# AbbVie-ComputationalGenomics/SAIGEgds

Measured on AMD Instinct MI355X. Metric: variants/sec seqAssocGLMM_SPA at N=430K; achieved HBM GB/s vs roofline, higher is better.
Workload: dtype f64

## Files before the change

### saigegds_amd/csrc/host_lanes.h

```cpp
extern "C" int sgx_set_option(sgx_handle *h, const char *name, long long value)
{
	if (!h || !name) return fail(SGX_EINVAL, "sgx_set_option: NULL argument");
	const std::string n(name);
	if (n == "score_v1") h->force_v1 = value != 0;
	else if (n == "force_dense") h->force_dense = value != 0;
	else if (n == "spa_exact") h->force_exact = value != 0;
	else if (n == "pipe_mb") { if (value < 0 || value > 65536) return fail(SGX_EINVAL, "pipe_mb out of range"); h->pipe_bytes = (size_t)value << 20; return SGX_OK; }
	else if (n == "spa_abl") h->spa_abl = (int)value;
	else if (n == "guard_exp") { if (value < 0 || value > 300) return fail(SGX_EINVAL, "guard_exp must be 0..300"); h->guard_tol = std::pow(10.0, -(double)value); }
	else if (n == "three_plane") { if (value < -1 || value > 1) return fail(SGX_EINVAL, "three_plane must be -1 (automatic), 0 or 1"); h->dense_opt = (int)value; return SGX_OK; }
	else if (n == "lanes") {
		if (value < 1 || value > 4) return fail(SGX_EINVAL, "lanes must be 1..4");
		if (h->owner) return fail(SGX_EINVAL, "lanes: not on a twin");
		int rc = sgx_sync(h);
		if (rc) return rc;
		for (int i = (int)value - 1; i < 3; i++) if (h->twins[i]) { sgx_free(h->twins[i]); h->twins[i] = nullptr; }
		for (int i = 0; i < (int)value - 1; i++) {
			if (h->twins[i]) continue;
			sgx_handle *t = new sgx_handle();
			t->device = h->device; t->md = h->md; t->mf_ok = h->mf_ok; t->mfe = h->mfe;
			for (int g = 0; g < MF_MAXG; g++) { t->mf[g] = h->mf[g]; t->mf_nbfv[g] = h->mf_nbfv[g]; }
			t->dF = h->dF; t->dX = h->dX; t->dy = h->dy; t->dmu = h->dmu; t->dmu2 = h->dmu2; t->dXM = h->dXM; t->dFl = h->dFl; t->dQ = h->dQ;
			t->shares_model = true; t->owner = h;
			t->force_dense = h->force_dense; t->force_v1 = h->force_v1; t->force_exact = h->force_exact;
			t->spa_abl = h->spa_abl; t->guard_tol = h->guard_tol;
			rc = set_dev(t);
			if (!rc) rc = alloc_workspace(t);
			if (rc) { sgx_free(t); return rc; }
			h->twins[i] = t;
		}
		h->n_lanes = (int)value; h->next_lane = 0; h->last_issued = nullptr;
		return SGX_OK;
	}
	else return fail(SGX_EINVAL, "sgx_set_option: unknown option '%s'", name);
	for (sgx_handle *t : h->twins) if (t) { int rc = sgx_set_option(t, name, value); if (rc) return rc; }
	return SGX_OK;
}

static void stats_add(sgx_stats &into, const sgx_stats &x)
{
	into.n_variants += x.n_variants; into.n_valid += x.n_valid; into.n_spa += x.n_spa;
	into.n_spa_dense += x.n_spa_dense; into.n_spa_slow += x.n_spa_slow;
	into.ms_score += x.ms_score; into.ms_spa += x.ms_spa; into.ms_total += x.ms_total;
	into.ms_kernel += x.ms_kernel; into.ms_lists += x.ms_lists;
	into.score_launches += x.score_launches; into.spa_launches += x.spa_launches;
	into.three_plane += x.three_plane; into.n_unlisted += x.n_unlisted; into.n_guarded += x.n_guarded;
}

static int sync_lane(sgx_handle *h)
{
	int rc = set_dev(h);
	if (rc) return rc;
	HIPCHK(hipStreamSynchronize(h->stream));
	if (h->pend_dense.active) {
		h->pend_dense.active = false;
		if (h->stats_pending && h->h_counters[2] > 0) {
			rc = launch_pending_dense(h);
			if (rc) return rc;
			HIPCHK(hipStreamSynchronize(h->stream));
		}
	}
	if (h->stats_pending) {
		h->stats.n_spa = (uint64_t)(h->h_counters[0] + h->h_counters[7] - h->h_counters[6] + h->h_counters[5]);
		h->stats.n_valid = (uint64_t)h->h_counters[1];
		h->stats.n_spa_dense = (uint64_t)h->h_counters[2];
		h->stats.n_spa_slow = (uint64_t)h->h_counters[4];
		h->stats.three_plane = h->form == FORM_THREE ? 1u : 0u;
		h->stats.n_guarded = (uint32_t)h->h_counters[21];
		h->stats.n_unlisted = (uint32_t)h->h_counters[23] - h->stats.n_guarded;
		if (h->form != FORM_FP64) {
			sgx_handle *p = h->owner ? h->owner : h;
			const double frac = 64.0 * (double)h->h_counters[22] / ((double)std::max<uint64_t>(1, h->stats.n_variants) * (double)h->md.N);
			const bool over = (uint64_t)h->stats.n_unlisted * 32 > h->stats.n_variants;
			if (h->form != FORM_THREE && (frac > SGX_DENSE_ON || over)) p->dense_mode = true;
			else if (h->form == FORM_THREE && frac < SGX_DENSE_OFF) p->dense_mode = false;
		}
#ifdef SPA5_PROF
		fprintf(stderr, "routing: tier A %d, tier B %d (of them handed on by A: %d), per-variant kernels %d (series list %d, exact list %d), dense %d\n",
			h->h_counters[0], h->h_counters[7], h->h_counters[6], h->h_counters[5], h->h_counters[3], h->h_counters[4], h->h_counters[2]);
		fprintf(stderr, "spa5 phases (10 ns ticks summed over variants): series kernel %d variants: stage %d count %d index %d gather %d series %d (sweep %d sum %d solve %d) | exact kernel %d variants: stage %d count %d index %d gather %d - sweeps %d\n",
			h->h_counters[3], h->h_counters[8], h->h_counters[9], h->h_counters[10], h->h_counters[11], h->h_counters[12], h->h_counters[13], h->h_counters[14], h->h_counters[15],
			h->h_counters[4], h->h_counters[16], h->h_counters[17], h->h_counters[18], h->h_counters[19], h->h_counters[21]);
#endif
		float a = 0, b = 0, c = 0;
		(void)hipEventElapsedTime(&a, h->ev[0], h->ev[1]);
		(void)hipEventElapsedTime(&b, h->ev[1], h->ev[2]);
		(void)hipEventElapsedTime(&c, h->ev[0], h->ev[2]);
		h->stats.ms_score = a; h->stats.ms_spa = b; h->stats.ms_total = c;
		float k = 0;
		if (h->evk_set) (void)hipEventElapsedTime(&k, h->evk[0], h->evk[1]);
		h->stats.ms_kernel = k; h->evk_set = false;
		float l = 0;
		if (h->lists_timed) { (void)hipEventElapsedTime(&l, h->ev_lists, h->ev[0]); h->stats.ms_total += l; }
		h->stats.ms_lists = l; h->lists_timed = false;
		h->stats_pending = false;
		sgx_handle *p = h->owner ? h->owner : h;
		stats_add(p->total, h->stats);
		p->total_calls++;
	}
	return SGX_OK;
}

extern "C" int sgx_sync(sgx_handle *h)
{
	if (!h) return fail(SGX_EINVAL, "sgx_sync: NULL handle");
	int rc = sync_lane(h);
	for (sgx_handle *t : h->twins) if (!rc && t) rc = sync_lane(t);
	return rc;
}

extern "C" int sgx_get_stats(sgx_handle *h, sgx_stats *st)
{
	if (!h || !st) return fail(SGX_EINVAL, "sgx_get_stats: NULL argument");
	int rc = sgx_sync(h);
	if (rc) return rc;
	*st = (h->last_issued && h->last_issued != h) ? h->last_issued->stats : h->stats;
	return SGX_OK;
}

extern "C" int sgx_get_stats_total(sgx_handle *h, sgx_stats *st, uint64_t *n_calls, int reset)
{
	if (!h || !st) return fail(SGX_EINVAL, "sgx_get_stats_total: NULL argument");
	int rc = sgx_sync(h);
	if (rc) return rc;
	*st = h->total;
	if (n_calls) *n_calls = h->total_calls;
	if (reset) { h->total = sgx_stats{}; h->total_calls = 0; }
	return SGX_OK;
}
```

### saigegds_amd/csrc/host_spa.h

```cpp


template <int LO, typename F, int... I>
static bool with_int(int v, F &&f, std::integer_sequence<int, I...>)
{
	return ((v == LO + I && (f(std::integral_constant<int, LO + I>()), true)) || ...);
}
template <typename F>
static bool with_k(int K, F &&f) { return with_int<1>(K, f, std::make_integer_sequence<int, KMAX>()); }
template <typename F>
static void with_pp(int P, F &&f)
{
	if (P <= 8) f(std::integral_constant<int, 8>());
	else if (P <= 16) f(std::integral_constant<int, 16>());
	else if (P <= 32) f(std::integral_constant<int, 32>());
	else f(std::integral_constant<int, 64>());
}

static dim3 mf_grid(int n_cu, size_t rows, int ntile, int *tps, int vpb = MF_VPB, int wg_per_cu = 2)
{
	const int vt = (int)((rows + vpb - 1) / vpb);
	int sk = std::max(1, (n_cu * wg_per_cu * 4 + vt / 2) / vt);
	sk = std::min(sk, std::max(1, ntile / 24));
	if (sk >= 6) sk = (sk + 7) & ~7;
	sk = std::min(sk, std::max(1, ntile / 2));
	*tps = (ntile + sk - 1) / sk;
	*tps += *tps & 1;
	sk = (ntile + *tps - 1) / *tps;
	return dim3((unsigned)vt, (unsigned)sk);
}

template <int KK, int NCX, int INPUT>
static const void *spa4_moments_fn()
{
	if constexpr (INPUT == IN_2BIT) return (const void *)spa4_moments<KK, NCX>;
	else return (const void *)spa4_moments_ds<KK, NCX, INPUT>;
}

template <int KK, int INPUT>
static int launch_spa_k(sgx_handle *h, RowsRef rr, size_t M, double *out8, bool lazy_dense)
{
	const DevModel &md = h->md;
	constexpr int PB = 512;
	hipStream_t st = h->stream;
	const dim3 sgrid((unsigned)std::min<size_t>(M, (size_t)h->spa_grid));
	if (h->force_v1 && INPUT != IN_2BIT) {
		hipLaunchKernelGGL((spa_kernel<KK, PB, INPUT>), sgrid, dim3(PB), 0, st, rr,
			md, h->recs, h->counters, 0, (const int *)nullptr, h->scratch, h->scratch_stride, out8);
		return SGX_OK;
	}
	const size_t fl = spa4_lds_bytes(KK);
	if (!h->mom_attr_set[INPUT]) {
		HIPCHK(hipFuncSetAttribute(spa4_moments_fn<KK, SPA4_NCA, INPUT>(), hipFuncAttributeMaxDynamicSharedMemorySize, (int)fl));
		HIPCHK(hipFuncSetAttribute(spa4_moments_fn<KK, SPA4_NCB, INPUT>(), hipFuncAttributeMaxDynamicSharedMemorySize, (int)fl));
		h->mom_attr_set[INPUT] = true;
	}
	const int nround = (int)((M + h->vcap4 - 1) / h->vcap4);
	const int btop = (int)(2 * M);
	const dim3 gsolve((unsigned)std::min((h->vcap4 + 3) / 4, 4 * h->n_cu));
	const size_t rowb5 = (size_t)((md.N + 63) / 64) * 16;
	const size_t l5 = (INPUT == IN_2BIT && rowb5 <= 120 * 1024) ? rowb5 : 0;
	const bool small5 = INPUT == IN_2BIT && rowb5 <= 32 * 1024;
	if (l5 > 48 * 1024 && !h->spa5_attr_set[INPUT]) {
		HIPCHK(hipFuncSetAttribute((const void *)spa5_kernel<KK, INPUT, 0, 512>, hipFuncAttributeMaxDynamicSharedMemorySize, (int)l5));
		HIPCHK(hipFuncSetAttribute((const void *)spa5_kernel<KK, INPUT, 1, 512>, hipFuncAttributeMaxDynamicSharedMemorySize, (int)l5));
		h->spa5_attr_set[INPUT] = true;
	}
	const int fx5 = (h->force_exact ? 1 : 0) | (h->spa_abl & ~1);
	auto moments = [&](auto ncx, int tier, int rd) {
		constexpr int NCX = decltype(ncx)::value;
		if constexpr (INPUT == IN_2BIT)
			hipLaunchKernelGGL((spa4_moments<KK, NCX>), dim3((unsigned)h->n_cu), dim3(WAVE * spa4_waves(KK)), fl, st, rr, md, h->nseg,
				tier, btop, rd * h->vcap4, h->vcap4, h->recs, h->counters, h->seg4, h->spa_abl, h->cur5 + 2);
		else
			hipLaunchKernelGGL((spa4_moments_ds<KK, NCX, INPUT>), dim3((unsigned)h->n_cu), dim3(WAVE * spa4_waves(KK)), fl, st,
				(const void *)rr.base, rr.bpv, md, h->nseg, tier, btop, rd * h->vcap4, h->vcap4, h->recs, h->counters, h->seg4, h->cur5 + 2);
		hipLaunchKernelGGL((spa4_solve<KK, NCX>), gsolve, dim3(256), 0, st, md, h->nseg, tier, btop, rd * h->vcap4, h->vcap4,
			h->recs, h->counters, h->seg4, h->fallback, h->fb_x2, out8, h->force_dense ? 1 : 0, h->force_exact ? 1 : 0);
	};
	for (int rd = 0; rd < nround; rd++) moments(std::integral_constant<int, SPA4_NCA>(), 0, rd);
	for (int rd = 0; rd < nround; rd++) moments(std::integral_constant<int, SPA4_NCB>(), 1, rd);
	const int only5 = (INPUT == IN_2BIT && rr.cptr != nullptr && (h->spa_abl & 512)) ? 2 : 0;
	const size_t ws5 = spa5_wg_bytes(md.N);
	auto spa5 = [&](auto threads, int nwg) {
		constexpr int T5 = decltype(threads)::value;
		if constexpr (T5 == 512 || INPUT == IN_2BIT) {
			hipLaunchKernelGGL((spa5_kernel<KK, INPUT, 0, T5>), dim3((unsigned)nwg), dim3(T5), l5, st, rr, md, h->recs, h->counters,
				h->fb_spa2, h->fb_x2, h->cur5, h->fallback, h->scr5, out8, h->force_dense ? 1 : 0, fx5, l5, only5, ws5, 3);
			hipLaunchKernelGGL((spa5_kernel<KK, INPUT, 1, T5>), dim3((unsigned)nwg), dim3(T5), l5, st, rr, md, h->recs, h->counters,
				h->fb_x2, h->fb_x2, h->cur5 + 1, h->fallback, h->scr5, out8, h->force_dense ? 1 : 0, fx5, l5, only5, ws5, 4);
		}
	};
	if (small5) spa5(std::integral_constant<int, 128>(), h->nwg5);
	else spa5(std::integral_constant<int, 512>(), h->n_cu);
	if (!lazy_dense)
		hipLaunchKernelGGL((spa_kernel<KK, PB, INPUT>), sgrid, dim3(PB), 0, st, rr,
			md, h->recs, h->counters, 2, h->fallback, h->scratch, h->scratch_stride, out8);
	return SGX_OK;
}

template <int INPUT>
static int launch_spa(sgx_handle *h, RowsRef rr, size_t M, double *out8, bool lazy_dense = false)
{
	h->stats.spa_launches = 0;
	if (h->md.quant) return SGX_OK;
	int rc = SGX_OK;
	with_k(h->md.K, [&](auto kk) { rc = launch_spa_k<decltype(kk)::value, INPUT>(h, rr, M, out8, lazy_dense); });
	if (rc) return rc;
	HIPCHK(hipGetLastError());
	const bool v1 = h->force_v1 && INPUT != IN_2BIT;
	h->stats.spa_launches = v1 ? 1u : (uint32_t)(4 * ((M + h->vcap4 - 1) / h->vcap4) + 3);
	if (lazy_dense && !v1) { h->pend_dense.active = true; h->pend_dense.rr = rr; h->pend_dense.M = M; h->pend_dense.out8 = out8; }
	return SGX_OK;
}

static int launch_pending_dense(sgx_handle *h)
{
	const dim3 sgrid((unsigned)std::min<size_t>(h->pend_dense.M, (size_t)h->spa_grid));
	with_k(h->md.K, [&](auto kk) {
		hipLaunchKernelGGL((spa_kernel<decltype(kk)::value, 512, IN_2BIT>), sgrid, dim3(512), 0, h->stream, h->pend_dense.rr, h->md,
			h->recs, h->counters, 2, h->fallback, h->scratch, h->scratch_stride, h->pend_dense.out8);
	});
	HIPCHK(hipGetLastError());
	return SGX_OK;
}

static int scan_begin(sgx_handle *h, hipStream_t sst, ScanForm form, const sgx_block *b)
{
	h->form = form;
	if (b) HIPCHK(hipStreamWaitEvent(sst, b->ready, 0));
	if (form == FORM_FP64) {
		HIPCHK(hipMemsetAsync(h->counters, 0, 24 * sizeof(int), sst));
		if (h->cur5) HIPCHK(hipMemsetAsync(h->cur5, 0, 8 * sizeof(int), sst));
	}
	HIPCHK(hipEventRecord(h->ev[0], sst));
	return SGX_OK;
}

template <int INPUT>
static int scan_end(sgx_handle *h, hipStream_t sst, const sgx_block *b, RowsRef rr, size_t M, double *out8, bool lazy_dense)
{
	HIPCHK(hipEventRecord(h->ev[1], sst));
	h->stats.score_launches = h->form == FORM_FP64 ? 1 : 5;
	if (sst != h->stream) HIPCHK(hipStreamWaitEvent(h->stream, h->ev[1], 0));
	int rc = launch_spa<INPUT>(h, rr, M, out8, lazy_dense);
	if (rc) return rc;
	if (lazy_dense) h->pend_dense.blk = b;
	HIPCHK(hipEventRecord(h->ev[2], h->stream));
	if (b) {
		HIPCHK(hipEventRecord(b->last_read, h->stream));
		const_cast<sgx_block *>(b)->was_read = true;
	}
	HIPCHK(hipMemcpyAsync(h->h_counters, h->counters, 24 * sizeof(int), hipMemcpyDeviceToHost, h->stream));
	h->stats.n_variants = M;
	h->stats_pending = true;
	return SGX_OK;
}

template <int KK, int INPUT>
static int launch_score_fp64(sgx_handle *h, RowsRef rr, size_t M, double *out8, uint8_t *valid)
{
	const DevModel &md = h->md;
	constexpr int SB = 256, P = 2 * KK + 2;
	hipStream_t st = h->stream;
	const dim3 grid((unsigned)M);
	if constexpr (INPUT == IN_2BIT) {
		hipLaunchKernelGGL((score2b_kernel<P, SB>), grid, dim3(SB), 0, st,
			rr, (int)M, md, h->recs, h->counters, out8, valid, (const int *)nullptr, 0, 0, (int *)nullptr, (int *)nullptr);
	} else {
		using T = std::conditional_t<INPUT == IN_U8, uint8_t, double>;
		const T *rows = reinterpret_cast<const T *>(rr.base);
		if constexpr (KK <= 8) {
			if (!h->force_v1) {
				const int vb = (int)((M + DS_TILE_VB - 1) / DS_TILE_VB);
				int ns = std::max(1, std::min((4 * h->n_cu + vb - 1) / vb, (md.N + 4095) / 4096));
				int per = (((md.N + ns - 1) / ns) + 63) & ~63;
				ns = (md.N + per - 1) / per;
				const size_t need = (size_t)ns * M * (3 * P + 2) * sizeof(double);
				if (need > h->ds_part_cap) {
					HIPCHK(hipStreamSynchronize(st));
					if (h->ds_part) HIPCHK(hipFree(h->ds_part));
					h->ds_part = nullptr; h->ds_part_cap = 0;
					HIPCHK(hipMalloc((void **)&h->ds_part, need));
					h->ds_part_cap = need;
				}
				hipLaunchKernelGGL((score_ds_tile_kernel<P, T>), dim3((unsigned)vb, (unsigned)ns), dim3(256), 0, st,
					rows, (int)M, md, per, h->ds_part);
				hipLaunchKernelGGL((score_ds_tile_epilogue<P>), dim3((unsigned)((M + 255) / 256)), dim3(256), 0, st,
					(int)M, md, ns, h->ds_part, h->recs, h->counters, out8, valid);
				return SGX_OK;
			}
		}
		hipLaunchKernelGGL((score_ds_kernel<P, SB, T>), grid, dim3(SB), 0, st, rows, (int)M, md, h->recs, h->counters, out8, valid);
	}
	return SGX_OK;
}

template <int INPUT>
static int launch_scan(sgx_handle *h, const void *rows, size_t row_bytes, size_t M, double *out8, uint8_t *valid,
	const sgx_block *b = nullptr)
{
	const RowsRef rr{reinterpret_cast<const uint8_t *>(rows), row_bytes, 0, nullptr, nullptr, nullptr};
	int rc = scan_begin(h, h->stream, FORM_FP64, b);
	if (rc) return rc;
	if (!with_k(h->md.K, [&](auto kk) { rc = launch_score_fp64<decltype(kk)::value, INPUT>(h, rr, M, out8, valid); }))
		return fail(SGX_EINVAL, "unsupported K=%d", h->md.K);
	if (rc) return rc;
	HIPCHK(hipGetLastError());
	return scan_end<INPUT>(h, h->stream, b, rr, M, out8, false);
}
```

### saigegds_amd/csrc/host_state.h

```cpp

struct sgx_block {
	int device = 0;
	int N = 0, ntile = 0, nr = 1;
	size_t cap = 0;
	size_t M = 0;
	bool lists_only = false;
	uint8_t *rows = nullptr;
	size_t bpv = 0;
	const uint8_t *ext_rows = nullptr; size_t ext_bpv = 0;
	unsigned *idx = nullptr; size_t idx_cap = 0;
	unsigned *cursor = nullptr;
	unsigned *lstart = nullptr;
	int *lcnt = nullptr;
	int *nzp = nullptr, *n2p = nullptr;
	int *n3 = nullptr;
	uint8_t *ovf = nullptr;
	int *nzv = nullptr, *n2v = nullptr;
	unsigned *cptr = nullptr;
	unsigned *cidx = nullptr;
	size_t cidx_cap = 0;
	uint8_t *corient = nullptr;
	hipEvent_t ready = nullptr;
	hipEvent_t last_read = nullptr;
	bool was_read = false;
	int *info = nullptr, *h_info = nullptr;
	bool info_read = false, dense = false;
};

enum ScanForm {
	FORM_FP64,
	FORM_LISTS,
	FORM_ROWS,
	FORM_THREE,
};

struct sgx_handle {
	int device = 0;
	hipStream_t stream = nullptr;
	DevModel md{};
	double *dF = nullptr, *dX = nullptr, *dy = nullptr, *dmu = nullptr, *dmu2 = nullptr, *dXM = nullptr;
	SpaRec *recs = nullptr; size_t recs_cap = 0;
	int *fallback = nullptr;
	int *fb_spa2 = nullptr;
	int *fb_x2 = nullptr;
	int nseg = 0;
	bool force_dense = false;
	double *seg4 = nullptr;
	int vcap4 = 0, nround4 = 0;
	bool spa5_attr_set[3] = {false, false, false};
	bool mom_attr_set[3] = {false, false, false};
	uint8_t *scr5 = nullptr; int *cur5 = nullptr; int nwg5 = 0;
	int spa_abl = 0;
	bool force_exact = false;
	bool mf_ok = false;
	MfTab mf[MF_MAXG]{};
	int mf_nbfv[MF_MAXG]{};
	MfEpi mfe{};
	uint8_t *dFl = nullptr;
	long long *dQ = nullptr;
	int *mf_acc = nullptr;
	int *s3_slabs = nullptr; size_t s3_slabs_cap = 0;
	long long *s3_t3 = nullptr; size_t s3_t3_cap = 0;
	int *s3_ovf = nullptr; size_t s3_ovf_cap = 0;
	bool s3_attr[17] = {false};
	bool s3_attr_miss[17] = {false};
	hipStream_t hstream = nullptr;
	hipStream_t s3_side = nullptr;
	hipEvent_t s3_fork = nullptr, s3_join = nullptr;
	sgx_block *tmp_blk[2] = {nullptr, nullptr};
	int n_cu = 256;
	int *counters = nullptr;
	int *h_counters = nullptr;
	double *scratch = nullptr; size_t scratch_stride = 0; int spa_grid = 0;
	uint8_t *stage_in = nullptr; size_t stage_in_cap = 0;
	hipStream_t cstream = nullptr;
	size_t pipe_bytes = 0;
	uint8_t *pipe_in[2] = {nullptr, nullptr}; size_t pipe_in_cap = 0;
	uint8_t *pipe_pk[2] = {nullptr, nullptr}; size_t pipe_pk_cap = 0;
	double *pipe_out[2] = {nullptr, nullptr}; uint8_t *pipe_valid[2] = {nullptr, nullptr}; size_t pipe_out_cap = 0;
	double *pin_out[2] = {nullptr, nullptr}; uint8_t *pin_valid[2] = {nullptr, nullptr};
	int *pipe_flag = nullptr, *h_pipe_flag = nullptr;
	hipEvent_t ev_h2d = nullptr;
	hipEvent_t ev_copy[2] = {nullptr, nullptr}, ev_done[2] = {nullptr, nullptr};
	uint8_t *stage_pk = nullptr; size_t stage_pk_cap = 0;
	double *ds_part = nullptr; size_t ds_part_cap = 0;
	double *stage_out = nullptr; uint8_t *stage_valid = nullptr; size_t stage_out_cap = 0;
	hipEvent_t ev[3] = {nullptr, nullptr, nullptr};
	hipEvent_t evk[2] = {nullptr, nullptr};
	bool evk_set = false;
	hipEvent_t ev_lists = nullptr;
	bool lists_timed = false;
	sgx_stats stats{};
	bool force_v1 = false;
	bool stats_pending = false;
	struct { bool active = false; RowsRef rr{}; size_t M = 0; double *out8 = nullptr; const sgx_block *blk = nullptr; } pend_dense;
	sgx_handle *twins[3] = {nullptr, nullptr, nullptr};
	int n_lanes = 1;
	sgx_handle *owner = nullptr;
	bool shares_model = false;
	bool dense_mode = false;
	int dense_opt = -1;
	double guard_tol = 2e-11;
	ScanForm form = FORM_FP64;
	int next_lane = 0;
	sgx_handle *last_issued = nullptr;
	sgx_stats total{};
	uint64_t total_calls = 0;
};

#define SGX_DENSE_ON  0.005
#define SGX_DENSE_OFF 0.003

static int set_dev(sgx_handle *h)
{
	HIPCHK(hipSetDevice(h->device));
	return SGX_OK;
}
```

### saigegds_amd/csrc/kern_spa4.h

```cpp
#pragma once
#include "kern_spa4_tab.h"


#ifndef SPA4_WAVES_LOWK
#define SPA4_WAVES_LOWK 8
#endif
__host__ __device__ constexpr int spa4_waves(int K) { return K <= 8 ? SPA4_WAVES_LOWK : 8; }
#define SPA4_NCA 12
#define SPA4_NCB SPA4_NC
#define SPA4_NSMAX (SPA4_NC + 5)
#define SPA4_TAIL_TOL 1e-10

__device__ __forceinline__ double spa4_fma_svv(double a_sgpr, double x, double c_vgpr)
{
	double r;
	asm("v_fma_f64 %0, %1, %2, %3" : "=v"(r) : "s"(a_sgpr), "v"(x), "v"(c_vgpr));
	return r;
}

__device__ __forceinline__ void spa4_max_abs(double &g, double a)
{
	asm("v_max_f64 %0, %0, |%1|" : "+v"(g) : "v"(a));
}

// ... 409 lines not shown
#pragma unroll
	for (int k = 1; k < NC - 3; k++) tp *= tau;
	const double tail = (fabs((double)(NC * (NC - 1)) * S.kp[NC - 3] * tp * tau) +
		fabs((double)((NC - 1) * (NC - 2)) * S.kp[NC - 4] * tp)) * its * its;
	return S.gmax * fabs(t) <= xmax && tail <= SPA4_TAIL_TOL * fabs(K2s) && isfinite(K2s);
}

template <int NC>
__device__ __forceinline__ bool spa4_root(const Spa4Series<NC> &S, double xmax, double q, double NAmu, double NAsigma, RootState &s)
{
	root_begin(s, q, 0, 0);
	root_feed(s, S.k1, S.k2, NAmu, NAsigma, 0.0, true);
	while (s.active) {
		double K1s, K2s, K0s;
		if (!spa4_eval(S, xmax, s.tnew, K1s, K2s, K0s)) return false;
		root_feed(s, K1s, K2s, NAmu, NAsigma, K0s, true);
	}
	return true;
}

template <int K, int NC>
__device__ __forceinline__ void spa4_solve_one(const DevModel &md, int nseg, int tier, int btop, int v0, int vcap, int v, int lane,
	SpaRec *__restrict__ recs, int *__restrict__ counters, const double *__restrict__ segpart,
	int *__restrict__ fb_dense, int *__restrict__ fb_exact, double *__restrict__ out8, int force_dense, int force_exact);

template <int K, int NC>
__global__ void __launch_bounds__(256)
spa4_solve(DevModel md, int nseg, int tier, int btop, int v0, int vcap, SpaRec *__restrict__ recs, int *__restrict__ counters,
	const double *__restrict__ segpart, int *__restrict__ fb_dense, int *__restrict__ fb_exact,
	double *__restrict__ out8, int force_dense, int force_exact)
{
	const int lane = threadIdx.x & (WAVE - 1);
	const int nflag = min(counters[tier ? 7 : 0] - v0, vcap);
	for (int v = (blockIdx.x * blockDim.x + threadIdx.x) / WAVE; v < nflag; v += gridDim.x * blockDim.x / WAVE)
		spa4_solve_one<K, NC>(md, nseg, tier, btop, v0, vcap, v, lane, recs, counters, segpart, fb_dense, fb_exact, out8,
			force_dense, force_exact);
}

template <int K, int NC>
__device__ __forceinline__ void spa4_solve_one(const DevModel &md, int nseg, int tier, int btop, int v0, int vcap, int v, int lane,
	SpaRec *__restrict__ recs, int *__restrict__ counters, const double *__restrict__ segpart,
	int *__restrict__ fb_dense, int *__restrict__ fb_exact, double *__restrict__ out8, int force_dense, int force_exact)
{
	constexpr int NS = NC + 5;
	const int ri = spa4_rec(tier, btop, v0 + v);
	const SpaRec r = recs[ri];
	double a[NS];
#pragma unroll
	for (int x = 0; x < NS; x++) a[x] = 0;
	for (int s = lane; s < nseg; s += WAVE) {
		const double *p = segpart + ((size_t)v * nseg + s) * NS;
#pragma unroll
		for (int x = 0; x < NS - 1; x++) a[x] += p[x];
		a[NS - 1] = fmax(a[NS - 1], p[NS - 1]);
	}
#pragma unroll
	for (int x = 0; x < NS - 1; x++) a[x] = wave_sum(a[x]);
#pragma unroll
	for (int o = 32; o > 0; o >>= 1) a[NS - 1] = fmax(a[NS - 1], __shfl_xor(a[NS - 1], o, WAVE));
	if (lane > 1) return;
	const double inv = 1 / sqrt(r.AC2);
	double xmu_c = 0, xsum_c = 0;
#pragma unroll
	for (int x = 0; x < K; x++) { xmu_c = fma(md.Xmu[x], r.c[x], xmu_c); xsum_c = fma(md.Xsum[x], r.c[x], xsum_c); }
	const double Tstat = r.S * inv;
	const double var2 = r.var2 / r.AC2, var1 = var2 * md.r;
	const double m1 = (a[0] - xmu_c) * inv;
	const double qtilde = Tstat / sqrt(var1) * sqrt(var2) + m1;
	const double sdev = qtilde - m1, qinv = -sdev + m1;
	const double pn_in = d_pchisq1_upper(sdev * sdev / var2);
	if (fabs(qtilde - m1) / sqrt(var2) < 2.0) {
		if (lane == 0) spa_write_row(r, Tstat, var1, pn_in, true, out8);
		return;
	}
	const double nb = (xsum_c - a[1]) * inv;
	const double L = a[2] + fmax(-nb, 0.0), U = a[3] + fmin(-nb, 0.0);
	const double mar = 1e-9 * (fabs(L) + fabs(U) + fabs(qtilde) + fabs(qinv));
	if (force_dense || !(qtilde < L - mar && qtilde > U + mar && qinv < L - mar && qinv > U + mar)) {
		if (lane == 0) fb_dense[atomicAdd(&counters[2], 1)] = ri;
		return;
	}
	Spa4Series<NC> S;
	S.k1 = a[4]; S.k2 = a[5]; S.ts = r.tscale; S.gmax = a[NS - 1];
#pragma unroll
	for (int x = 0; x < NC - 2; x++) S.kp[x] = a[6 + x];
	const double NAmu = m1 - a[4], NAsigma = var2 - a[5];
	const double qmine = lane == 0 ? qtilde : qinv;
	RootState sm;
	const bool ok_mine = !force_exact && spa4_root(S, md.spa_xmax, qmine, NAmu, NAsigma, sm);
	double p_mine = 0;
	if (ok_mine && sm.converged) p_mine = lugannani_rice(sm.root, sm.Kcur, sm.K2cur, qmine, NAmu, NAsigma);
	const int st_mine = (ok_mine ? 1 : 0) | (ok_mine && sm.converged ? 2 : 0);
	const double p_other = __shfl(p_mine, 1, WAVE);
	const int st_other = __shfl(st_mine, 1, WAVE);
	if (lane != 0) return;
	if (!(st_mine & 1) || !(st_other & 1)) {
		if (tier == 0 && !force_exact) {
			const int slot = atomicAdd(&counters[7], 1);
			atomicAdd(&counters[6], 1);
			recs[btop - 1 - slot] = r;
		} else {
			fb_exact[atomicAdd(&counters[4], 1)] = ri;
		}
		return;
	}
	double pval;
	bool converged = true;
	if ((st_mine & 2) && (st_other & 2)) {
		pval = fabs(p_mine) + fabs(p_other);
		if (pval != 0 && pn_in / pval > 1000) pval = pn_in;
	} else {
		pval = pn_in;
		converged = false;
	}
	spa_write_row(r, Tstat, var1, pval, converged, out8);
}


#define SPA5_BIG 2048

__device__ __forceinline__ void cgf_terms_rt(double g, double m, double t, bool with_k, double &k1, double &k2, double &k0)
{
	const double om = 1 - m, mg = m * g, c2 = om * mg * g;
	const double e = fast_exp(-g * t);
	const double d = fma(om, e, m);
	const double rr = isfinite(d) ? fast_rcp(d) : 0.0;
	k1 = fma(mg, rr, k1);
	const double tt = c2 * e * rr * rr;
	if (isfinite(tt)) k2 += tt;
	if (with_k) k0 += cgf_korg_term(g, m, t, d, om);
}

__host__ __device__ inline size_t spa5_wg_bytes(int N) { return (((size_t)N + 63) & ~(size_t)63) * (16 + 4); }

template <int BLOCK>
__device__ __noinline__ void spa5_cum_sweep(const double2 *__restrict__ glist, int nnz, double ts, double *kp_out)
{
	constexpr int NC = SPA4_NCB;
	double kp[NC - 1];
#pragma unroll
	for (int a = 0; a < NC - 1; a++) kp[a] = 0;
	double2 gn = (int)threadIdx.x < nnz ? glist[threadIdx.x] : make_double2(0.0, 0.5);
	for (int k = threadIdx.x; k < nnz; k += BLOCK) {
		const double2 gm = gn;
		if (k + BLOCK < nnz) gn = glist[k + BLOCK];
		const double mui = gm.y;
		spa4_cum_terms<NC>(gm.x * ts, mui * (1 - mui), 1 - 2 * mui, kp);
		kp[NC - 2] = fmax(kp[NC - 2], fabs(gm.x));
	}
#pragma unroll
	for (int a = 0; a < NC - 1; a++) kp_out[a] = kp[a];
}

__device__ __noinline__ int spa5_series_solve(const double *arg, const SpaRec *__restrict__ rec, double *__restrict__ out8)
{
	constexpr int NC = SPA4_NCB;
	Spa4Series<NC> S;
#pragma unroll
	for (int a = 0; a < NC - 2; a++) S.kp[a] = arg[a];
	S.k1 = arg[NC - 2]; S.k2 = arg[NC - 1]; S.ts = arg[NC]; S.gmax = arg[NC + 1];
	const double xmax = arg[NC + 2], qtilde = arg[NC + 3], qinv = arg[NC + 4], NAmu = arg[NC + 5], NAsigma = arg[NC + 6];
	const double pn_in = arg[NC + 7], Tstat = arg[NC + 8], var1 = arg[NC + 9];
	RootState s1, s2;
	if (!spa4_root(S, xmax, qtilde, NAmu, NAsigma, s1) || !spa4_root(S, xmax, qinv, NAmu, NAsigma, s2)) return 0;
	double pval;
	bool converged = true;
	if (s1.converged && s2.converged) {
		const double p1 = lugannani_rice(s1.root, s1.Kcur, s1.K2cur, qtilde, NAmu, NAsigma);
		const double p2 = lugannani_rice(s2.root, s2.Kcur, s2.K2cur, qinv, NAmu, NAsigma);
		pval = fabs(p1) + fabs(p2);
		if (pval != 0 && pn_in / pval > 1000) pval = pn_in;
	} else {
		pval = pn_in;
		converged = false;
	}
	const SpaRec rr = *rec;
	spa_write_row(rr, Tstat, var1, pval, converged, out8);
	return 1;
}

template <int BLOCK>
__device__ __forceinline__ bool spa5_series(const double2 *__restrict__ glist, int nnz, double ts, double xmax,
	double k1, double k2, double qtilde, double qinv, double NAmu, double NAsigma, double pn_in,
	double Tstat, double var1, const SpaRec *__restrict__ rec, double *__restrict__ out8, double *sh, int *sh_flag, int *prof = nullptr)
{
	constexpr int NC = SPA4_NCB;
	double kp[NC - 1];
#ifdef SPA5_PROF
	long long tp_ = wall_clock64();
#define SPA5_TS(ph) do { if (threadIdx.x == 0) { const long long now_ = wall_clock64(); atomicAdd(&prof[ph], (int)(now_ - tp_)); tp_ = now_; } } while (0)
#else
#define SPA5_TS(ph) do { } while (0)
#endif
	spa5_cum_sweep<BLOCK>(glist, nnz, ts, kp);
	SPA5_TS(0);
	constexpr int NWV = BLOCK / WAVE;
	double gmax = kp[NC - 2];
	const int lane = threadIdx.x & (WAVE - 1), wv = threadIdx.x / WAVE;
	double kr[NC - 2];
#pragma unroll
	for (int a = 0; a < NC - 2; a++) kr[a] = kp[a];
	const int idx = wave_reduce_scatter(kr, lane);
#pragma unroll
	for (int o = 32; o > 0; o >>= 1) gmax = fmax(gmax, __shfl_xor(gmax, o, WAVE));
	double *part = sh + NC + 16;
	if (!(lane & 3) && idx < NC - 2) part[idx * NWV + wv] = kr[0];
	if (lane == 1) part[(NC - 2) * NWV + wv] = gmax;
	__syncthreads();
	double *arg = sh;
	if (threadIdx.x < NC - 2) {
		double t = 0;
		for (int w = 0; w < NWV; w++) t += part[threadIdx.x * NWV + w];
		arg[threadIdx.x] = t;
	}
	__syncthreads();
	SPA5_TS(1);
	if (threadIdx.x == 0) {
		for (int w = 0; w < NWV; w++) gmax = fmax(gmax, part[(NC - 2) * NWV + w]);
		arg[NC - 2] = k1; arg[NC - 1] = k2; arg[NC] = ts; arg[NC + 1] = gmax; arg[NC + 2] = xmax;
		arg[NC + 3] = qtilde; arg[NC + 4] = qinv; arg[NC + 5] = NAmu; arg[NC + 6] = NAsigma;
		arg[NC + 7] = pn_in; arg[NC + 8] = Tstat; arg[NC + 9] = var1;
		*sh_flag = spa5_series_solve(arg, rec, out8);
	}
	SPA5_TS(2);
	__syncthreads();
	const bool done = *sh_flag != 0;
	__syncthreads();
	return done;
}

#ifndef SPA5_REG_WAVES
#define SPA5_REG_WAVES 2
#endif
#define SPA5_WAVES_PER_SIMD(BLOCK) ((BLOCK) == 512 ? SPA5_REG_WAVES : ((BLOCK) / 64 + 3) / 4)
#ifdef SPA5_PROF
#define SPA5_T(ph) do { if (tid == 0) { const long long now_ = wall_clock64(); atomicAdd(&counters[8 + 8 * MODE + (ph)], (int)(now_ - tprev_)); tprev_ = now_; } } while (0)
#else
#define SPA5_T(ph) do { } while (0)
#endif
template <int K, int INPUT, int MODE, int BLOCK>
__global__ void __launch_bounds__(BLOCK, SPA5_WAVES_PER_SIMD(BLOCK))
spa5_kernel(RowsRef rr, DevModel md, const SpaRec *__restrict__ recs,
	int *__restrict__ counters, const int *__restrict__ todo, int *__restrict__ todo_next, int *__restrict__ cursor,
	int *__restrict__ fb_dense, uint8_t *__restrict__ scratch, double *__restrict__ out8, int force_dense, int force_exact,
	size_t lds_row_bytes, int only, size_t wg_stride, int nslot)
{
	constexpr int KP = (K + 2) & ~1, NW = BLOCK / WAVE;
	extern __shared__ __attribute__((aligned(16))) uint8_t fill_smem[];
	uint4 *rows_lds = reinterpret_cast<uint4 *>(fill_smem);
	__shared__ double sh[SPA4_NCB * NW + SPA4_NCB + 16];
	__shared__ int sh_flag;
	__shared__ int shi[NW];
	__shared__ int sh_vi, sh_v;
	__shared__ SpaRec sh_rec;
	const int N = md.N, tid = threadIdx.x, lane = tid & (WAVE - 1), wid = tid / WAVE;
	double2 *glist = reinterpret_cast<double2 *>(scratch + (size_t)blockIdx.x * wg_stride);
	uint32_t *ilist = reinterpret_cast<uint32_t *>(glist + (((size_t)N + 63) & ~(size_t)63));
	const int ntodo = counters[nslot];
	const int nvec = INPUT == IN_2BIT ? (int)(min((size_t)((N + 63) >> 6) * 16, rr_row_bytes(rr)) / 16) : (N + 63) >> 6;
	const int per = ((nvec + NW - 1) / NW + WAVE - 1) & ~(WAVE - 1);
	for (;;) {
		__syncthreads();
		if (tid < WAVE) {
			int vi0 = 0;
			if (tid == 0) vi0 = atomicAdd(cursor, 1);
			vi0 = __builtin_amdgcn_readfirstlane(vi0);
			int v0 = -1;
			if (vi0 < 2 * ntodo) {
				v0 = todo[vi0 < ntodo ? vi0 : vi0 - ntodo];
				const double *src = reinterpret_cast<const double *>(recs + v0);
				for (int i = tid; i < (int)(sizeof(SpaRec) / 8); i += WAVE) reinterpret_cast<double *>(&sh_rec)[i] = src[i];
			}
			if (tid == 0) { sh_vi = vi0; sh_v = v0; }
		}
		__syncthreads();
		const int vi = sh_vi;
		if (vi >= 2 * ntodo) break;
#ifdef SPA5_PROF
		long long tprev_ = wall_clock64();
#endif
		const bool big_round = vi < ntodo;
		const int v = sh_v;
		const SpaRec &r = sh_rec;
		if ((r.nnz > SPA5_BIG) != big_round) continue;
		auto row_piece = [&](int p) -> uint4 { return *reinterpret_cast<const uint4 *>(rr.base + rr_piece(rr, (size_t)r.j, (size_t)p)); };
		const uint32_t zx = r.minus ? 0xAAAAAAAAu : 0u;
		const double lut0 = r.lut[0], lut1 = r.lut[1], lut2 = r.lut[2], lut3 = r.lut[3];
		const bool listed = INPUT == IN_2BIT && only != 2 && rr.cptr != nullptr && rr.corient[r.j] == (r.minus ? 2 : 1);
		const uint32_t *il = listed ? rr.cidx + rr.cptr[r.j] : ilist;
		int nnz = listed ? r.nnz : 0;
		if (!listed) {
			const bool staged = INPUT == IN_2BIT && lds_row_bytes >= (size_t)nvec * 16;
			if (staged) {
				constexpr int UN = 8;
				for (int p0 = tid; p0 < nvec; p0 += UN * BLOCK) {
					uint4 t[UN];
	#pragma unroll
					for (int j = 0; j < UN; j++) { const int p = p0 + j * BLOCK; t[j] = p < nvec ? row_piece(p) : make_uint4(0u, 0u, 0u, 0u); }
	#pragma unroll
					for (int j = 0; j < UN; j++) { const int p = p0 + j * BLOCK; if (p < nvec) rows_lds[p] = t[j]; }
				}
				__syncthreads();
			}
			SPA5_T(0);
			auto masks = [&](int p, uint32_t (&ww)[4], uint32_t (&z)[4]) -> int {
				int cnt = 0;
				if (INPUT == IN_2BIT) {
					uint4 w = make_uint4(0u, 0u, 0u, 0u);
					if (p < nvec) w = staged ? rows_lds[p] : row_piece(p);
					ww[0] = w.x; ww[1] = w.y; ww[2] = w.z; ww[3] = w.w;
	#pragma unroll
					for (int k = 0; k < 4; k++) { z[k] = nz_fields((ww[k] ^ zx) & keep_mask(N - p * 64 - 16 * k)); cnt += __popc(z[k]); }
				} else {
					z[0] = z[1] = z[2] = z[3] = 0;
					if (p < nvec) {
						for (int s2 = 0; s2 < 64; s2++) {
							const int i = p * 64 + s2;
							if (i < N && load_dosage<INPUT>(rr, i, r) != 0) { z[s2 >> 5] |= 1u << (s2 & 31); cnt++; }
						}
					}
				}
				return cnt;
			};
			int cnt_w = 0;
			for (int it = 0; it < per; it += WAVE) {
				uint32_t ww[4], z[4];
				cnt_w += masks(wid * per + it + lane, ww, z);
			}
			cnt_w = wave_sum_i(cnt_w);
			if (lane == 0) shi[wid] = cnt_w;
			__syncthreads();
			int o_w = 0;
	#pragma unroll
			for (int w = 0; w < NW; w++) { if (w < wid) o_w += shi[w]; nnz += shi[w]; }
			SPA5_T(1);
			for (int it = 0; it < per; it += WAVE) {
				uint32_t ww[4], z[4];
				const int p = wid * per + it + lane;
				const int cnt = masks(p, ww, z);
				if (!__ballot(cnt != 0)) continue;
				int incl = cnt;
	#pragma unroll
				for (int o = 1; o < WAVE; o <<= 1) {
					const int up = __shfl_up(incl, o, WAVE);
					if (lane >= o) incl += up;
				}
				int o2 = o_w + incl - cnt;
				o_w += __shfl(incl, WAVE - 1, WAVE);
				if (INPUT == IN_2BIT) {
	#pragma unroll
					for (int k = 0; k < 4; k++) {
						uint32_t zz = z[k];
						while (zz) {
							const int b = __ffs(zz) - 1;
							zz &= zz - 1;
							ilist[o2++] = (uint32_t)(p * 64 + 16 * k + (b >> 1)) | (((ww[k] >> b) & 3u) << 30);
						}
					}
				} else {
	#pragma unroll
					for (int k = 0; k < 2; k++) {
						uint32_t zz = z[k];
						while (zz) {
							const int b = __ffs(zz) - 1;
							zz &= zz - 1;
							ilist[o2++] = (uint32_t)(p * 64 + 32 * k + b);
						}
					}
				}
			}
			__syncthreads();
			SPA5_T(2);
		}
		const double inv = 1 / sqrt(r.AC2);
		double c[K];
#pragma unroll
		for (int a = 0; a < K; a++) c[a] = r.c[a];
		double a6[6] = {0, 0, 0, 0, 0, 0};
		constexpr int UNG = K <= 4 ? 4 : 2;
		for (int k0 = tid; k0 < ((force_exact & 128) ? 0 : nnz); k0 += UNG * BLOCK) {
			uint32_t e[UNG];
			double xv[UNG][KP];
#pragma unroll
			for (int j = 0; j < UNG; j++) e[j] = (k0 + j * BLOCK < nnz) ? il[k0 + j * BLOCK] : 0u;
#pragma unroll
			for (int j = 0; j < UNG; j++) {
				const double *x = md.XM + (size_t)(e[j] & 0x3FFFFFFFu) * KP;
#pragma unroll
				for (int a = 0; a < KP; a += 2) {
					const double2 t2 = *reinterpret_cast<const double2 *>(x + a);
					xv[j][a] = t2.x; xv[j][a + 1] = t2.y;
				}
			}
#pragma unroll
			for (int j = 0; j < UNG; j++) {
				const int k = k0 + j * BLOCK;
				if (k >= nnz) continue;
				const uint32_t code = e[j] >> 30;
				const double G = INPUT == IN_2BIT ? ((code & 2u) ? ((code & 1u) ? lut3 : lut2) : ((code & 1u) ? lut1 : lut0))
					: load_dosage<INPUT>(rr, (int)(e[j] & 0x3FFFFFFFu), r);
				double b = 0;
#pragma unroll
				for (int a = 0; a < K; a++) b = fma(xv[j][a], c[a], b);
				const double mui = xv[j][K];
				const double adj = (G - b) * inv;
				glist[k] = make_double2(adj, mui);
				a6[0] = fma(mui, G, a6[0]);
				a6[1] += b;
				if (adj > 0) a6[2] += adj; else a6[3] += adj;
				a6[4] = fma(adj, mui, a6[4]);
				a6[5] = fma(adj * adj, mui * (1 - mui), a6[5]);
			}
		}
		block_sum<6, BLOCK>(a6, sh);
		SPA5_T(3);
		double xmu_c = 0, xsum_c = 0;
#pragma unroll
		for (int a = 0; a < K; a++) { xmu_c = fma(md.Xmu[a], c[a], xmu_c); xsum_c = fma(md.Xsum[a], c[a], xsum_c); }
		const double m1 = (a6[0] - xmu_c) * inv;
		const double Tstat = r.S * inv;
		const double var2 = r.var2 / r.AC2, var1 = var2 * md.r;
		const double qtilde = Tstat / sqrt(var1) * sqrt(var2) + m1;
		const double sdev = qtilde - m1, qinv = -sdev + m1;
		const double pn_in = d_pchisq1_upper(sdev * sdev / var2);
		double pval;
		bool converged = true;
		if (fabs(qtilde - m1) / sqrt(var2) < 2.0) {
			pval = pn_in;
		} else {
			const double nb = (xsum_c - a6[1]) * inv;
			const double L = a6[2] + fmax(-nb, 0.0), U = a6[3] + fmin(-nb, 0.0);
			const double mar = 1e-9 * (fabs(L) + fabs(U) + fabs(qtilde) + fabs(qinv));
			if (force_dense || !(qtilde < L - mar && qtilde > U + mar && qinv < L - mar && qinv > U + mar)) {
				if (tid == 0) fb_dense[atomicAdd(&counters[2], 1)] = v;
				continue;
			}
			const double NAmu = m1 - a6[4], NAsigma = var2 - a6[5];
			if (MODE == 0) {
				if ((force_exact & 1) || !spa5_series<BLOCK>(glist, nnz, r.tscale, md.spa_xmax, a6[4], a6[5], qtilde, qinv, NAmu, NAsigma,
						pn_in, Tstat, var1, &sh_rec, out8, sh, &sh_flag, counters + 13)) {
					if (tid == 0) todo_next[atomicAdd(&counters[4], 1)] = v;
				}
				SPA5_T(4);
				continue;
			}
			RootState s1, s2;
			root_begin(s1, qtilde, L, U);
			root_begin(s2, qinv, L, U);
			root_feed(s1, a6[4], a6[5], NAmu, NAsigma, 0.0, true);
			root_feed(s2, a6[4], a6[5], NAmu, NAsigma, 0.0, true);
			auto sweep = [&](bool a1, bool a2, bool k1w, bool k2w, double t1, double t2, double (&sv)[6]) {
#pragma unroll
				for (int a = 0; a < 6; a++) sv[a] = 0;
				double2 gn = tid < nnz ? glist[tid] : make_double2(0.0, 0.5);
				for (int k0 = tid; k0 < nnz; k0 += BLOCK) {
					const double2 gm = gn;
					if (k0 + BLOCK < nnz) gn = glist[k0 + BLOCK];
					if (a1) cgf_terms_rt(gm.x, gm.y, t1, k1w, sv[0], sv[1], sv[2]);
					if (a2) cgf_terms_rt(gm.x, gm.y, t2, k2w, sv[3], sv[4], sv[5]);
				}
				block_sum<6, BLOCK>(sv, sh);
			};
			while ((s1.active || s2.active) && !(force_exact & 64)) {
				const bool a1 = s1.active, a2 = s2.active, k1w = s1.want_k, k2w = s2.want_k;
				double sv[6];
				sweep(a1, a2, k1w, k2w, s1.tnew, s2.tnew, sv);
				if (a1) root_feed(s1, sv[0], sv[1], NAmu, NAsigma, sv[2], k1w);
				if (a2) root_feed(s2, sv[3], sv[4], NAmu, NAsigma, sv[5], k2w);
			}
			if (s1.converged && s2.converged) {
				if (!(s1.k_ok && s2.k_ok)) {
					double sv[6];
					sweep(!s1.k_ok, !s2.k_ok, true, true, s1.root, s2.root, sv);
					if (!s1.k_ok) s1.Kcur = sv[2];
					if (!s2.k_ok) s2.Kcur = sv[5];
				}
				const double p1 = lugannani_rice(s1.root, s1.Kcur, s1.K2cur, qtilde, NAmu, NAsigma);
				const double p2 = lugannani_rice(s2.root, s2.Kcur, s2.K2cur, qinv, NAmu, NAsigma);
				pval = fabs(p1) + fabs(p2);
				if (pval != 0 && pn_in / pval > 1000) pval = pn_in;
			} else {
				pval = pn_in;
				converged = false;
			}
		}
		if (tid == 0) spa_write_row(r, Tstat, var1, pval, converged, out8);
		SPA5_T(5);
	}
}
```

Baseline: 18.50 million.

## Fuse SPA5 series and exact passes into one kernel with LDS-resident glist

```diff
diff --git a/saigegds_amd/csrc/host_lanes.h b/saigegds_amd/csrc/host_lanes.h
--- a/saigegds_amd/csrc/host_lanes.h
+++ b/saigegds_amd/csrc/host_lanes.h
@@ -5,6 +5,7 @@
 	if (n == "score_v1") h->force_v1 = value != 0;
 	else if (n == "force_dense") h->force_dense = value != 0;
 	else if (n == "spa_exact") h->force_exact = value != 0;
+	else if (n == "spa5_split") h->spa5_split = value != 0;
 	else if (n == "pipe_mb") { if (value < 0 || value > 65536) return fail(SGX_EINVAL, "pipe_mb out of range"); h->pipe_bytes = (size_t)value << 20; return SGX_OK; }
 	else if (n == "spa_abl") h->spa_abl = (int)value;
 	else if (n == "guard_exp") { if (value < 0 || value > 300) return fail(SGX_EINVAL, "guard_exp must be 0..300"); h->guard_tol = std::pow(10.0, -(double)value); }
@@ -22,7 +23,7 @@
 			for (int g = 0; g < MF_MAXG; g++) { t->mf[g] = h->mf[g]; t->mf_nbfv[g] = h->mf_nbfv[g]; }
 			t->dF = h->dF; t->dX = h->dX; t->dy = h->dy; t->dmu = h->dmu; t->dmu2 = h->dmu2; t->dXM = h->dXM; t->dFl = h->dFl; t->dQ = h->dQ;
 			t->shares_model = true; t->owner = h;
-			t->force_dense = h->force_dense; t->force_v1 = h->force_v1; t->force_exact = h->force_exact;
+			t->force_dense = h->force_dense; t->force_v1 = h->force_v1; t->force_exact = h->force_exact; t->spa5_split = h->spa5_split;
 			t->spa_abl = h->spa_abl; t->guard_tol = h->guard_tol;
 			rc = set_dev(t);
 			if (!rc) rc = alloc_workspace(t);
@@ -64,7 +65,7 @@
 		h->stats.n_spa = (uint64_t)(h->h_counters[0] + h->h_counters[7] - h->h_counters[6] + h->h_counters[5]);
 		h->stats.n_valid = (uint64_t)h->h_counters[1];
 		h->stats.n_spa_dense = (uint64_t)h->h_counters[2];
-		h->stats.n_spa_slow = (uint64_t)h->h_counters[4];
+		h->stats.n_spa_slow = (uint64_t)(h->h_counters[4] + h->h_counters[20]);
 		h->stats.three_plane = h->form == FORM_THREE ? 1u : 0u;
 		h->stats.n_guarded = (uint32_t)h->h_counters[21];
 		h->stats.n_unlisted = (uint32_t)h->h_counters[23] - h->stats.n_guarded;
diff --git a/saigegds_amd/csrc/host_spa.h b/saigegds_amd/csrc/host_spa.h
--- a/saigegds_amd/csrc/host_spa.h
+++ b/saigegds_amd/csrc/host_spa.h
@@ -63,6 +63,8 @@
 	if (l5 > 48 * 1024 && !h->spa5_attr_set[INPUT]) {
 		HIPCHK(hipFuncSetAttribute((const void *)spa5_kernel<KK, INPUT, 0, 512>, hipFuncAttributeMaxDynamicSharedMemorySize, (int)l5));
 		HIPCHK(hipFuncSetAttribute((const void *)spa5_kernel<KK, INPUT, 1, 512>, hipFuncAttributeMaxDynamicSharedMemorySize, (int)l5));
+		if constexpr (INPUT == IN_2BIT)
+			HIPCHK(hipFuncSetAttribute((const void *)spa5_kernel<KK, INPUT, 2, 512>, hipFuncAttributeMaxDynamicSharedMemorySize, (int)l5));
 		h->spa5_attr_set[INPUT] = true;
 	}
 	const int fx5 = (h->force_exact ? 1 : 0) | (h->spa_abl & ~1);
@@ -83,6 +85,13 @@
 	const size_t ws5 = spa5_wg_bytes(md.N);
 	auto spa5 = [&](auto threads, int nwg) {
 		constexpr int T5 = decltype(threads)::value;
+		if constexpr (INPUT == IN_2BIT) {
+			if (!h->spa5_split) {
+				hipLaunchKernelGGL((spa5_kernel<KK, INPUT, 2, T5>), dim3((unsigned)nwg), dim3(T5), l5, st, rr, md, h->recs, h->counters,
+					h->fb_spa2, h->fb_x2, h->cur5, h->fallback, h->scr5, out8, h->force_dense ? 1 : 0, fx5, l5, only5, ws5, 3);
+				return;
+			}
+		}
 		if constexpr (T5 == 512 || INPUT == IN_2BIT) {
 			hipLaunchKernelGGL((spa5_kernel<KK, INPUT, 0, T5>), dim3((unsigned)nwg), dim3(T5), l5, st, rr, md, h->recs, h->counters,
 				h->fb_spa2, h->fb_x2, h->cur5, h->fallback, h->scr5, out8, h->force_dense ? 1 : 0, fx5, l5, only5, ws5, 3);
@@ -108,7 +117,8 @@
 	if (rc) return rc;
 	HIPCHK(hipGetLastError());
 	const bool v1 = h->force_v1 && INPUT != IN_2BIT;
-	h->stats.spa_launches = v1 ? 1u : (uint32_t)(4 * ((M + h->vcap4 - 1) / h->vcap4) + 3);
+	const unsigned n5 = (INPUT == IN_2BIT && !h->spa5_split) ? 1u : 2u;
+	h->stats.spa_launches = v1 ? 1u : (uint32_t)(4 * ((M + h->vcap4 - 1) / h->vcap4) + n5 + 1);
 	if (lazy_dense && !v1) { h->pend_dense.active = true; h->pend_dense.rr = rr; h->pend_dense.M = M; h->pend_dense.out8 = out8; }
 	return SGX_OK;
 }
diff --git a/saigegds_amd/csrc/host_state.h b/saigegds_amd/csrc/host_state.h
--- a/saigegds_amd/csrc/host_state.h
+++ b/saigegds_amd/csrc/host_state.h
@@ -52,6 +52,7 @@
 	uint8_t *scr5 = nullptr; int *cur5 = nullptr; int nwg5 = 0;
 	int spa_abl = 0;
 	bool force_exact = false;
+	bool spa5_split = true;
 	bool mf_ok = false;
 	MfTab mf[MF_MAXG]{};
 	int mf_nbfv[MF_MAXG]{};
diff --git a/saigegds_amd/csrc/kern_spa4.h b/saigegds_amd/csrc/kern_spa4.h
--- a/saigegds_amd/csrc/kern_spa4.h
+++ b/saigegds_amd/csrc/kern_spa4.h
@@ -585,6 +585,26 @@
 	for (int a = 0; a < NC - 1; a++) kp_out[a] = kp[a];
 }
 
+typedef const __attribute__((address_space(3))) double *spa5_lds_list;
+__device__ __forceinline__ double2 spa5_lds_at(spa5_lds_list g, int k) { return make_double2(g[2 * k], g[2 * k + 1]); }
+
+template <int BLOCK>
+__device__ __noinline__ void spa5_cum_sweep_lds(spa5_lds_list glist, int nnz, double ts, double *kp_out)
+{
+	constexpr int NC = SPA4_NCB;
+	double kp[NC - 1];
+#pragma unroll
+	for (int a = 0; a < NC - 1; a++) kp[a] = 0;
+	for (int k = threadIdx.x; k < nnz; k += BLOCK) {
+		const double2 gm = spa5_lds_at(glist, k);
+		const double mui = gm.y;
+		spa4_cum_terms<NC>(gm.x * ts, mui * (1 - mui), 1 - 2 * mui, kp);
+		kp[NC - 2] = fmax(kp[NC - 2], fabs(gm.x));
+	}
+#pragma unroll
+	for (int a = 0; a < NC - 1; a++) kp_out[a] = kp[a];
+}
+
 __device__ __noinline__ int spa5_series_solve(const double *arg, const SpaRec *__restrict__ rec, double *__restrict__ out8)
 {
 	constexpr int NC = SPA4_NCB;
@@ -615,7 +635,8 @@
 template <int BLOCK>
 __device__ __forceinline__ bool spa5_series(const double2 *__restrict__ glist, int nnz, double ts, double xmax,
 	double k1, double k2, double qtilde, double qinv, double NAmu, double NAsigma, double pn_in,
-	double Tstat, double var1, const SpaRec *__restrict__ rec, double *__restrict__ out8, double *sh, int *sh_flag, int *prof = nullptr)
+	double Tstat, double var1, const SpaRec *__restrict__ rec, double *__restrict__ out8, double *sh, int *sh_flag, int *prof = nullptr,
+	bool in_lds = false, spa5_lds_list glds = nullptr)
 {
 	constexpr int NC = SPA4_NCB;
 	double kp[NC - 1];
@@ -625,7 +646,8 @@
 #else
 #define SPA5_TS(ph) do { } while (0)
 #endif
-	spa5_cum_sweep<BLOCK>(glist, nnz, ts, kp);
+	if (in_lds) spa5_cum_sweep_lds<BLOCK>(glds, nnz, ts, kp);
+	else spa5_cum_sweep<BLOCK>(glist, nnz, ts, kp);
 	SPA5_TS(0);
 	constexpr int NWV = BLOCK / WAVE;
 	double gmax = kp[NC - 2];
@@ -667,7 +689,7 @@
 #endif
 #define SPA5_WAVES_PER_SIMD(BLOCK) ((BLOCK) == 512 ? SPA5_REG_WAVES : ((BLOCK) / 64 + 3) / 4)
 #ifdef SPA5_PROF
-#define SPA5_T(ph) do { if (tid == 0) { const long long now_ = wall_clock64(); atomicAdd(&counters[8 + 8 * MODE + (ph)], (int)(now_ - tprev_)); tprev_ = now_; } } while (0)
+#define SPA5_T(ph) do { if (tid == 0) { const long long now_ = wall_clock64(); atomicAdd(&counters[8 + 8 * (MODE == 1 || (MODE == 2 && (ph) == 5)) + (ph)], (int)(now_ - tprev_)); tprev_ = now_; } } while (0)
 #else
 #define SPA5_T(ph) do { } while (0)
 #endif
@@ -684,12 +706,15 @@
 	__shared__ double sh[SPA4_NCB * NW + SPA4_NCB + 16];
 	__shared__ int sh_flag;
 	__shared__ int shi[NW];
-	__shared__ int sh_vi, sh_v;
+	__shared__ int sh_vi, sh_v, sh_x;
 	__shared__ SpaRec sh_rec;
 	const int N = md.N, tid = threadIdx.x, lane = tid & (WAVE - 1), wid = tid / WAVE;
 	double2 *glist = reinterpret_cast<double2 *>(scratch + (size_t)blockIdx.x * wg_stride);
 	uint32_t *ilist = reinterpret_cast<uint32_t *>(glist + (((size_t)N + 63) & ~(size_t)63));
-	const int ntodo = counters[nslot];
+	const int n_x = MODE == 2 ? counters[4] : 0;
+	const int ntodo = MODE == 2 ? counters[3] + n_x : counters[nslot];
+	spa5_lds_list glds = (spa5_lds_list)(fill_smem);
+	__attribute__((address_space(3))) double *glds_w = (__attribute__((address_space(3))) double *)(fill_smem);
 	const int nvec = INPUT == IN_2BIT ? (int)(min((size_t)((N + 63) >> 6) * 16, rr_row_bytes(rr)) / 16) : (N + 63) >> 6;
 	const int per = ((nvec + NW - 1) / NW + WAVE - 1) & ~(WAVE - 1);
 	for (;;) {
@@ -698,13 +723,15 @@
 			int vi0 = 0;
 			if (tid == 0) vi0 = atomicAdd(cursor, 1);
 			vi0 = __builtin_amdgcn_readfirstlane(vi0);
-			int v0 = -1;
+			int v0 = -1, x0 = 0;
 			if (vi0 < 2 * ntodo) {
-				v0 = todo[vi0 < ntodo ? vi0 : vi0 - ntodo];
+				const int qi = vi0 < ntodo ? vi0 : vi0 - ntodo;
+				x0 = qi < n_x;
+				v0 = x0 ? todo_next[qi] : todo[qi - n_x];
 				const double *src = reinterpret_cast<const double *>(recs + v0);
 				for (int i = tid; i < (int)(sizeof(SpaRec) / 8); i += WAVE) reinterpret_cast<double *>(&sh_rec)[i] = src[i];
 			}
-			if (tid == 0) { sh_vi = vi0; sh_v = v0; }
+			if (tid == 0) { sh_vi = vi0; sh_v = v0; sh_x = x0; }
 		}
 		__syncthreads();
 		const int vi = sh_vi;
@@ -714,6 +741,7 @@
 #endif
 		const bool big_round = vi < ntodo;
 		const int v = sh_v;
+		const bool routed_exact = MODE == 2 && sh_x != 0;
 		const SpaRec &r = sh_rec;
 		if ((r.nnz > SPA5_BIG) != big_round) continue;
 		auto row_piece = [&](int p) -> uint4 { return *reinterpret_cast<const uint4 *>(rr.base + rr_piece(rr, (size_t)r.j, (size_t)p)); };
@@ -805,6 +833,7 @@
 			__syncthreads();
 			SPA5_T(2);
 		}
+		const bool in_lds = MODE == 2 && __builtin_amdgcn_readfirstlane((int)((size_t)nnz * 16 <= lds_row_bytes)) != 0;
 		const double inv = 1 / sqrt(r.AC2);
 		double c[K];
 #pragma unroll
@@ -837,7 +866,8 @@
 				for (int a = 0; a < K; a++) b = fma(xv[j][a], c[a], b);
 				const double mui = xv[j][K];
 				const double adj = (G - b) * inv;
-				glist[k] = make_double2(adj, mui);
+				if (in_lds) { glds_w[2 * k] = adj; glds_w[2 * k + 1] = mui; }
+				else glist[k] = make_double2(adj, mui);
 				a6[0] = fma(mui, G, a6[0]);
 				a6[1] += b;
 				if (adj > 0) a6[2] += adj; else a6[3] += adj;
@@ -869,13 +899,15 @@
 				continue;
 			}
 			const double NAmu = m1 - a6[4], NAsigma = var2 - a6[5];
-			if (MODE == 0) {
-				if ((force_exact & 1) || !spa5_series<BLOCK>(glist, nnz, r.tscale, md.spa_xmax, a6[4], a6[5], qtilde, qinv, NAmu, NAsigma,
-						pn_in, Tstat, var1, &sh_rec, out8, sh, &sh_flag, counters + 13)) {
-					if (tid == 0) todo_next[atomicAdd(&counters[4], 1)] = v;
+			if (MODE == 0 || (MODE == 2 && !routed_exact)) {
+				const bool done = !(force_exact & 1) && spa5_series<BLOCK>(glist, nnz, r.tscale, md.spa_xmax, a6[4], a6[5], qtilde, qinv,
+					NAmu, NAsigma, pn_in, Tstat, var1, &sh_rec, out8, sh, &sh_flag, counters + 13, in_lds, glds);
+				if (!done && tid == 0) {
+					if (MODE == 0) todo_next[atomicAdd(&counters[4], 1)] = v;
+					else atomicAdd(&counters[20], 1);
 				}
 				SPA5_T(4);
-				continue;
+				if (MODE == 0 || done) continue;
 			}
 			RootState s1, s2;
 			root_begin(s1, qtilde, L, U);
@@ -885,12 +917,20 @@
 			auto sweep = [&](bool a1, bool a2, bool k1w, bool k2w, double t1, double t2, double (&sv)[6]) {
 #pragma unroll
 				for (int a = 0; a < 6; a++) sv[a] = 0;
-				double2 gn = tid < nnz ? glist[tid] : make_double2(0.0, 0.5);
-				for (int k0 = tid; k0 < nnz; k0 += BLOCK) {
-					const double2 gm = gn;
-					if (k0 + BLOCK < nnz) gn = glist[k0 + BLOCK];
-					if (a1) cgf_terms_rt(gm.x, gm.y, t1, k1w, sv[0], sv[1], sv[2]);
-					if (a2) cgf_terms_rt(gm.x, gm.y, t2, k2w, sv[3], sv[4], sv[5]);
+				if (in_lds) {
+					for (int k0 = tid; k0 < nnz; k0 += BLOCK) {
+						const double2 gm = spa5_lds_at(glds, k0);
+						if (a1) cgf_terms_rt(gm.x, gm.y, t1, k1w, sv[0], sv[1], sv[2]);
+						if (a2) cgf_terms_rt(gm.x, gm.y, t2, k2w, sv[3], sv[4], sv[5]);
+					}
+				} else {
+					double2 gn = tid < nnz ? glist[tid] : make_double2(0.0, 0.5);
+					for (int k0 = tid; k0 < nnz; k0 += BLOCK) {
+						const double2 gm = gn;
+						if (k0 + BLOCK < nnz) gn = glist[k0 + BLOCK];
+						if (a1) cgf_terms_rt(gm.x, gm.y, t1, k1w, sv[0], sv[1], sv[2]);
+						if (a2) cgf_terms_rt(gm.x, gm.y, t2, k2w, sv[3], sv[4], sv[5]);
+					}
 				}
 				block_sum<6, BLOCK>(sv, sh);
 			};
```

After: 17.94 million. 3.0% lower.
